# Fadi987/PL-BERT

Measured on AMD Instinct MI355X. Metric: phoneme-tokens/sec, higher is better.
Workload: dtype bf16; 1 GPU; PL-BERT masked-phoneme training step (fwd+loss+bwd+allreduce+AdamW), ALBERT hidden 768 / 12 shared layers / FFN 2048 / 12 heads, seq_len 512, batch 32 per GPU; global_batch=32, seq_len=512, parallelism=dp1

## Files before the change

### plbert_amd/_lib.py

```python
from __future__ import annotations

import ctypes as C
import os

import torch

HERE = os.path.dirname(os.path.abspath(__file__))
LIB_PATH = os.environ.get("PLBERT_HIP_LIB") or os.path.join(HERE, "libplbert_hip.so")

PLB_PARAM_NAMES = [
    "encoder.embeddings.word_embeddings.weight",
    "encoder.embeddings.position_embeddings.weight",
    "encoder.embeddings.token_type_embeddings.weight",
    "encoder.embeddings.LayerNorm.weight",
    "encoder.embeddings.LayerNorm.bias",
    "encoder.encoder.embedding_hidden_mapping_in.weight",
    "encoder.encoder.embedding_hidden_mapping_in.bias",
    "encoder.encoder.albert_layer_groups.0.albert_layers.0.full_layer_layer_norm.weight",
    "encoder.encoder.albert_layer_groups.0.albert_layers.0.full_layer_layer_norm.bias",
    "encoder.encoder.albert_layer_groups.0.albert_layers.0.attention.query.weight",
    "encoder.encoder.albert_layer_groups.0.albert_layers.0.attention.key.weight",
    "encoder.encoder.albert_layer_groups.0.albert_layers.0.attention.value.weight",
    "encoder.encoder.albert_layer_groups.0.albert_layers.0.attention.query.bias",
    "encoder.encoder.albert_layer_groups.0.albert_layers.0.attention.key.bias",
    "encoder.encoder.albert_layer_groups.0.albert_layers.0.attention.value.bias",
    "encoder.encoder.albert_layer_groups.0.albert_layers.0.attention.dense.weight",
    "encoder.encoder.albert_layer_groups.0.albert_layers.0.attention.dense.bias",
    "encoder.encoder.albert_layer_groups.0.albert_layers.0.attention.LayerNorm.weight",
    "encoder.encoder.albert_layer_groups.0.albert_layers.0.attention.LayerNorm.bias",
    "encoder.encoder.albert_layer_groups.0.albert_layers.0.ffn.weight",
    "encoder.encoder.albert_layer_groups.0.albert_layers.0.ffn.bias",
    "encoder.encoder.albert_layer_groups.0.albert_layers.0.ffn_output.weight",
    "encoder.encoder.albert_layer_groups.0.albert_layers.0.ffn_output.bias",
    "phoneme_predictor.weight",
    "phoneme_predictor.bias",
    "encoder.pooler.weight",
    "encoder.pooler.bias",
    "token_predictor.weight",
    "token_predictor.bias",
]
PLB_NPARAM = len(PLB_PARAM_NAMES)

PUBLIC_SYMBOLS = [
    "plb_last_error", "plb_create", "plb_destroy", "plb_param_layout", "plb_workspace_bytes", "plb_bind",
    "plb_sync_weights", "plb_forward", "plb_pooler", "plb_loss_fwd_bwd", "plb_loss_fwd", "plb_loss_fwd_bwd_dual", "plb_adamw_step",
    "plb_set_fp8", "plb_fp8_state", "plb_fp8_stats", "plb_token_head_steps", "plb_set_token_head_steps", "plb_comm_unique_id", "plb_comm_init", "plb_comm_destroy",
    "plb_comm_info", "plb_comm_pieces", "plb_last_application_rows", "plb_status", "plb_status_ex", "plb_poll_status", "plb_status_export", "plb_status_import", "plb_broadcast_params", "plb_set_grad_overlap", "plb_allreduce_grads", "plb_apply_mask",
    "plb_mask_batch", "plb_profile_enable", "plb_profile_num_classes", "plb_profile_class_name", "plb_profile_read",
    "plb_debug_skip_piece", "plb_debug_ln_fault", "plb_debug_hb_audit", "plb_debug_hb_report", "plb_comm_trace", "plb_comm_trace_read",
    "plb_set_gemm_nt_tile", "plb_set_gemm_nt_prefetch", "plb_set_attn_bwd_fused", "plb_set_prune_last",
]


class PlbConfig(C.Structure):
    _fields_ = [
        ("vocab_size", C.c_int32), ("embedding_size", C.c_int32), ("hidden_size", C.c_int32),
        ("num_attention_heads", C.c_int32), ("intermediate_size", C.c_int32), ("num_hidden_layers", C.c_int32),
        ("max_position_embeddings", C.c_int32), ("type_vocab_size", C.c_int32), ("layer_norm_eps", C.c_float),
        ("num_phonemes", C.c_int32), ("num_tokens", C.c_int32), ("max_batch", C.c_int32), ("max_seq", C.c_int32),
        ("inference_only", C.c_int32),
    ]


class PlbGemmNT(C.Structure):
    _fields_ = [
        ("A", C.c_void_p), ("lda", C.c_int), ("B", C.c_void_p), ("ldb", C.c_int),
        ("M", C.c_int), ("N", C.c_int), ("K", C.c_int), ("Mstore", C.c_int),
        ("bias", C.c_void_p), ("res", C.c_void_p), ("ldr", C.c_int), ("aux", C.c_void_p), ("ldaux", C.c_int),
        ("C", C.c_void_p), ("ldc", C.c_int), ("C2", C.c_void_p), ("ldc2", C.c_int), ("Cf", C.c_void_p), ("ldcf", C.c_int),
        ("colpart", C.c_void_p),
        ("ce_cols", C.c_int), ("ce_tgt", C.c_void_p), ("ce_pmax", C.c_void_p), ("ce_psum", C.c_void_p),
        ("ce_tlogit", C.c_void_p), ("ce_lse", C.c_void_p), ("ce_w", C.c_void_p),
        ("deq_a", C.c_void_p), ("deq_b", C.c_void_p), ("C8", C.c_void_p), ("ldc8", C.c_int), ("q_scale", C.c_void_p),
        ("q_amax", C.c_void_p), ("c8_bf8", C.c_int),
        ("ln_gamma", C.c_void_p), ("ln_beta", C.c_void_p), ("ln_mean", C.c_void_p), ("ln_rstd", C.c_void_p),
        ("ln_eps", C.c_float), ("ln_xchg", C.c_void_p), ("ln_err", C.c_void_p), ("ln_fault", C.c_int),
    ]


class PlbGemmTN(C.Structure):
    _fields_ = [
        ("A", C.c_void_p), ("lda", C.c_int), ("Ncols", C.c_int), ("B", C.c_void_p), ("ldb", C.c_int),
        ("Mtot", C.c_int), ("N", C.c_int), ("K", C.c_int), ("rows_per_split", C.c_int), ("splits", C.c_int),
        ("slab", C.c_void_p), ("deq_a", C.c_void_p), ("deq_b", C.c_void_p),
    ]


class PlbAttn(C.Structure):
    _fields_ = [
        ("qkv", C.c_void_p), ("ldqkv", C.c_int), ("lengths", C.c_void_p),
        ("B", C.c_int), ("S", C.c_int), ("NH", C.c_int), ("H", C.c_int), ("scale", C.c_float),
        ("ctx", C.c_void_p), ("ldctx", C.c_int), ("lse", C.c_void_p),
        ("dctx", C.c_void_p), ("lddctx", C.c_int), ("delta", C.c_void_p), ("dqkv", C.c_void_p), ("lddqkv", C.c_int),
        ("colpart", C.c_void_p), ("colpart_accumulate", C.c_int),
        ("ctx8", C.c_void_p), ("ldctx8", C.c_int), ("ctx_scale", C.c_void_p), ("ctx_amax", C.c_void_p),
        ("dqkv8", C.c_void_p), ("lddqkv8", C.c_int), ("dqkv_scale", C.c_void_p), ("dqkv_amax", C.c_void_p),
        ("qoff", C.c_void_p), ("q", C.c_void_p), ("ldq", C.c_int), ("nq_total", C.c_int), ("dq", C.c_void_p), ("lddq", C.c_int),
        ("dq8", C.c_void_p), ("lddq8", C.c_int),
    ]


class PlbEmbed(C.Structure):
    _fields_ = [
        ("ids", C.c_void_p), ("T", C.c_int), ("S", C.c_int), ("E", C.c_int), ("V", C.c_int),
        ("word", C.c_void_p), ("pos", C.c_void_p), ("type0", C.c_void_p), ("gamma", C.c_void_p), ("beta", C.c_void_p),
        ("eps", C.c_float), ("out", C.c_void_p), ("ldo", C.c_int), ("dout", C.c_void_p), ("lddo", C.c_int),
        ("dx", C.c_void_p), ("dword", C.c_void_p), ("dpos", C.c_void_p), ("partials", C.c_void_p), ("nblocks", C.c_int),
    ]


class PlbLayerNorm(C.Structure):
    _fields_ = [
        ("x", C.c_void_p), ("ldx", C.c_int), ("gamma", C.c_void_p), ("beta", C.c_void_p), ("eps", C.c_float),
        ("y", C.c_void_p), ("ldy", C.c_int), ("mean", C.c_void_p), ("rstd", C.c_void_p),
        ("T", C.c_int), ("H", C.c_int), ("Tzero", C.c_int),
        ("dy", C.c_void_p), ("lddy", C.c_int), ("dx", C.c_void_p), ("lddx", C.c_int),
        ("partials", C.c_void_p), ("nblocks", C.c_int), ("accumulate", C.c_int),
        ("out8", C.c_void_p), ("ld8", C.c_int), ("q_scale", C.c_void_p), ("q_amax", C.c_void_p),
    ]


_lib = None


class HipLibraryMissing(RuntimeError):
    pass


def lib():
    global _lib
    if _lib is not None:
        return _lib
    if not os.path.exists(LIB_PATH):
        raise HipLibraryMissing(
            f"{LIB_PATH} is missing: build it with `python -m plbert_amd.build` (needs hipcc, gfx950). "
            "There is no CPU fallback for the PL-BERT hot path.")
    try:
        L = C.CDLL(LIB_PATH, mode=C.RTLD_GLOBAL)
    except OSError as ex:
        raise HipLibraryMissing(f"cannot load {LIB_PATH}: {ex}") from ex
    vp, i32, i64p, f32, f64 = C.c_void_p, C.c_int32, C.POINTER(C.c_int64), C.c_float, C.c_double
    L.plb_last_error.restype = C.c_char_p
    L.plb_last_error.argtypes = []
    L.plb_create.restype = C.c_int
    L.plb_create.argtypes = [C.POINTER(PlbConfig), C.POINTER(vp)]
    L.plb_destroy.restype = None
    L.plb_destroy.argtypes = [vp]
    L.plb_param_layout.restype = C.c_int
    L.plb_param_layout.argtypes = [vp, i64p, i64p, i64p, i64p]
    L.plb_workspace_bytes.restype = C.c_int64
    L.plb_workspace_bytes.argtypes = [vp]
    L.plb_bind.restype = C.c_int
    L.plb_bind.argtypes = [vp, vp, vp, vp, vp, vp, C.c_int64]
    L.plb_sync_weights.restype = C.c_int
    L.plb_sync_weights.argtypes = [vp, vp]
    L.plb_forward.restype = C.c_int
    L.plb_forward.argtypes = [vp, vp, vp, i32, i32, vp, vp, vp, vp]
    L.plb_loss_fwd_bwd.restype = C.c_int
    L.plb_loss_fwd_bwd.argtypes = [vp, vp, vp, vp, vp, vp, i32, i32, i32, vp, vp]
    L.plb_loss_fwd_bwd_dual.restype = C.c_int
    L.plb_loss_fwd_bwd_dual.argtypes = [vp, vp, vp, vp, vp, vp, vp, i32, i32, i32, vp, vp, vp]
    L.plb_pooler.restype = C.c_int
    L.plb_pooler.argtypes = [vp, vp, i32, i32, vp, vp]
    L.plb_loss_fwd.restype = C.c_int
    L.plb_loss_fwd.argtypes = [vp, vp, vp, vp, vp, vp, vp, i32, i32, i32, vp, vp, vp]
    L.plb_set_fp8.restype = C.c_int
    L.plb_set_fp8.argtypes = [vp, i32, vp]
    L.plb_fp8_state.restype = C.c_int
    L.plb_fp8_state.argtypes = [vp, C.POINTER(i32), C.POINTER(i32)]
    L.plb_token_head_steps.restype = i32
    L.plb_token_head_steps.argtypes = [vp]
    L.plb_set_token_head_steps.restype = C.c_int
    L.plb_set_token_head_steps.argtypes = [vp, i32]
    L.plb_comm_unique_id.restype = C.c_int
    L.plb_comm_unique_id.argtypes = [vp]
    L.plb_comm_init.restype = C.c_int
    L.plb_comm_init.argtypes = [vp, vp, i32, i32]
    L.plb_comm_destroy.restype = C.c_int
    L.plb_comm_destroy.argtypes = [vp]
    L.plb_comm_info.restype = C.c_int
    L.plb_comm_info.argtypes = [vp, C.POINTER(i32), C.POINTER(i32), C.POINTER(i32)]
    L.plb_status.restype = C.c_int
    L.plb_status.argtypes = [vp, C.POINTER(i32)]
    L.plb_status_ex.restype = C.c_int
    L.plb_status_ex.argtypes = [vp, C.POINTER(i32), C.POINTER(i32)]
    L.plb_poll_status.restype = C.c_int
    L.plb_poll_status.argtypes = [vp, C.POINTER(i32)]
    L.plb_fp8_stats.restype = C.c_int
    L.plb_fp8_stats.argtypes = [vp, C.POINTER(f32), C.POINTER(f32), vp]
    L.plb_last_application_rows.restype = C.c_int
    L.plb_last_application_rows.argtypes = [vp, i64p, i64p]
    L.plb_status_export.restype = C.c_int
    L.plb_status_export.argtypes = [vp, vp, vp]
    L.plb_status_import.restype = C.c_int
    L.plb_status_import.argtypes = [vp, vp, vp]
    L.plb_debug_hb_audit.restype = C.c_int
    L.plb_debug_hb_audit.argtypes = [vp, i32, i32]
    L.plb_debug_hb_report.restype = C.c_int
    L.plb_debug_hb_report.argtypes = [vp, i64p, C.POINTER(i32), C.c_char_p, i32]
    L.plb_comm_trace.restype = C.c_int
    L.plb_comm_trace.argtypes = [vp, i32]
    L.plb_comm_trace_read.restype = C.c_int
    L.plb_comm_trace_read.argtypes = [vp, i32, C.POINTER(i32), i64p, i64p, C.POINTER(f32), C.POINTER(f32), C.POINTER(f32)]
    L.plb_debug_ln_fault.restype = None
    L.plb_debug_ln_fault.argtypes = [C.c_int, C.c_int]
    L.plb_debug_skip_piece.restype = None
    L.plb_debug_skip_piece.argtypes = [C.c_int]
    L.plb_comm_pieces.restype = C.c_int
    L.plb_comm_pieces.argtypes = [vp, C.POINTER(i32), C.POINTER(C.c_int64)]
    L.plb_broadcast_params.restype = C.c_int
    L.plb_broadcast_params.argtypes = [vp, i32, vp]
    L.plb_set_grad_overlap.restype = C.c_int
    L.plb_set_grad_overlap.argtypes = [vp, i32]
    L.plb_allreduce_grads.restype = C.c_int
    L.plb_allreduce_grads.argtypes = [vp, vp]
    L.plb_apply_mask.restype = C.c_int
    L.plb_apply_mask.argtypes = [vp, vp, vp, vp, vp, vp, vp, vp, C.c_int64, vp, i32, i32, i32, vp, vp, vp, vp, vp, vp, vp, vp]
    L.plb_adamw_step.restype = C.c_int
    L.plb_adamw_step.argtypes = [vp, f64, f64, f64, f64, f64, i32, f64, vp]
    L.plb_mask_batch.restype = C.c_int
    L.plb_mask_batch.argtypes = [vp, vp, i32, i32, C.c_uint64, C.c_uint32, f32, f32, f32, i32, i32, vp, vp, vp, vp, vp]
    L.plb_profile_enable.restype = None
    L.plb_profile_enable.argtypes = [C.c_int]
    L.plb_profile_num_classes.restype = C.c_int
    L.plb_profile_num_classes.argtypes = []
    L.plb_profile_class_name.restype = C.c_char_p
    L.plb_profile_class_name.argtypes = [C.c_int]
    L.plb_profile_read.restype = C.c_int
    L.plb_profile_read.argtypes = [C.POINTER(C.c_double), i64p, C.POINTER(C.c_double), C.POINTER(C.c_double)]
    L.plb_launch_gemm_nt.restype = C.c_int
    L.plb_launch_gemm_nt.argtypes = [C.POINTER(PlbGemmNT), C.c_int, C.c_int, vp]
    L.plb_set_gemm_nt_tile.restype = None
    L.plb_set_gemm_nt_tile.argtypes = [C.c_int]
    L.plb_set_gemm_nt_prefetch.restype = None
    L.plb_set_gemm_nt_prefetch.argtypes = [C.c_int]
    L.plb_launch_gemm_nt_fp8.restype = C.c_int
    L.plb_launch_gemm_nt_fp8.argtypes = [C.POINTER(PlbGemmNT), C.c_int, C.c_int, vp]
    L.plb_launch_gemm_nt_fp8_ln.restype = C.c_int
    L.plb_launch_gemm_nt_fp8_ln.argtypes = [C.POINTER(PlbGemmNT), C.c_int, C.c_int, vp]
    L.plb_launch_gemm_nt_fp8_gelud.restype = C.c_int
    L.plb_launch_gemm_nt_fp8_gelud.argtypes = [C.POINTER(PlbGemmNT), C.c_int, C.c_int, vp]
    L.plb_launch_gemm_tn.restype = C.c_int
    L.plb_launch_gemm_tn.argtypes = [C.POINTER(PlbGemmTN), vp]
    L.plb_launch_gemm_tn_big.restype = C.c_int
    L.plb_launch_gemm_tn_big.argtypes = [C.POINTER(PlbGemmTN), vp]
    L.plb_launch_gemm_tn_fp8.restype = C.c_int
    L.plb_launch_gemm_tn_fp8.argtypes = [C.POINTER(PlbGemmTN), vp]
    L.plb_launch_reduce_slabs.restype = C.c_int
    L.plb_launch_reduce_slabs.argtypes = [vp, C.c_int, C.c_size_t, vp, C.c_int, vp]
    L.plb_launch_attn_fwd.restype = C.c_int
    L.plb_launch_attn_fwd.argtypes = [C.POINTER(PlbAttn), vp]
    L.plb_launch_gemm_nt_ln.restype = C.c_int
    L.plb_launch_gemm_nt_ln.argtypes = [C.POINTER(PlbGemmNT), C.c_int, vp]
    L.plb_launch_gemm_nt_gelud.restype = C.c_int
    L.plb_launch_gemm_nt_gelud.argtypes = [C.POINTER(PlbGemmNT), C.c_int, vp]
    L.plb_launch_attn_bwd.restype = C.c_int
    L.plb_launch_attn_bwd.argtypes = [C.POINTER(PlbAttn), vp]
    L.plb_launch_attn_bwd_fused.restype = C.c_int
    L.plb_launch_attn_bwd_fused.argtypes = [C.POINTER(PlbAttn), vp]
    L.plb_set_prune_last.restype = None
    L.plb_set_prune_last.argtypes = [C.c_int]
    L.plb_set_attn_bwd_fused.restype = None
    L.plb_set_attn_bwd_fused.argtypes = [C.c_int]
    L.plb_launch_ln_fwd.restype = C.c_int
    L.plb_launch_ln_fwd.argtypes = [C.POINTER(PlbLayerNorm), vp]
    L.plb_launch_ln_bwd.restype = C.c_int
    L.plb_launch_ln_bwd.argtypes = [C.POINTER(PlbLayerNorm), vp]
    L.plb_launch_embed_scatter.restype = C.c_int
    L.plb_launch_embed_scatter.argtypes = [C.POINTER(PlbEmbed), C.c_int, vp]
    L.plb_launch_colsum.restype = C.c_int
    L.plb_launch_colsum.argtypes = [vp, C.c_int, C.c_size_t, C.c_int, C.c_int, vp, C.c_int, C.c_int, vp, C.c_int, vp]
    _lib = L
    return L


def profile_enable(on):
    lib().plb_profile_enable(int(bool(on)))


def profile_read():
    L = lib()
    n = L.plb_profile_num_classes()
    ms, fl, by = (C.c_double * n)(), (C.c_double * n)(), (C.c_double * n)()
    cnt = (C.c_int64 * n)()
    check(L.plb_profile_read(ms, cnt, fl, by), "plb_profile_read")
    return {L.plb_profile_class_name(i).decode(): dict(ms=ms[i], launches=int(cnt[i]), flops=fl[i], bytes=by[i])
            for i in range(n) if cnt[i]}


def check(rc, what):
    if rc != 0:
        msg = lib().plb_last_error().decode("utf-8", "replace")
        raise RuntimeError(f"{what} failed: {msg or 'rc=%d' % rc}")
```

### plbert_amd/build.py

```python
from __future__ import annotations

import os
import subprocess
import sys

HERE = os.path.dirname(os.path.abspath(__file__))
CSRC = os.path.join(HERE, "csrc")
LIB = os.path.join(HERE, "libplbert_hip.so")
SOURCES = ["gemm.hip", "gemm_big.hip", "gemm_fp8.hip", "gemm_fp8_ln.hip", "gemm_tn_fp8.hip", "gemm_ln.hip", "attn.hip", "attn_bwd_fused.hip", "rowops.hip", "mask.hip", "engine.cpp"]
HEADERS = ["common.h", "plbert_kernels.h", "gemm_epilogue.h", "gemm_nt_pipeline.h", "attn_common.h", os.path.join("..", "..", "include", "plbert.h")]
FLAGS = ["--offload-arch=gfx950", "-O3", "-std=c++17", "-fPIC", "-Wall", "-Wno-unused-function"]
_NO_SINK = ["-mllvm", "-disable-machine-sink"]
EXTRA_FLAGS = {"attn_bwd_fused.hip": ["-mllvm", "-amdgpu-mfma-vgpr-form=1"],
               "gemm_fp8.hip": _NO_SINK, "gemm_fp8_ln.hip": _NO_SINK, "gemm_tn_fp8.hip": _NO_SINK}


def _hipcc():
    for cand in (os.environ.get("HIPCC"), "/opt/rocm/bin/hipcc", "hipcc"):
        if cand and (os.path.isabs(cand) and os.path.exists(cand) or not os.path.isabs(cand)):
            return cand
    raise RuntimeError("hipcc not found")


def needs_build():
    if not os.path.exists(LIB):
        return True
    t = os.path.getmtime(LIB)
    deps = [os.path.join(CSRC, s) for s in SOURCES + HEADERS]
    return any(os.path.getmtime(d) > t for d in deps)


OBJDUMP = "/opt/rocm/lib/llvm/bin/llvm-objdump"


def disassemble_code_objects(lib, workdir):
    import glob
    import shutil
    cp = shutil.copy(lib, workdir)
    subprocess.run([OBJDUMP, "--offloading", cp], check=True, stdout=subprocess.PIPE, stderr=subprocess.STDOUT)
    cos = sorted(glob.glob(cp + ".*gfx950"))
    if not cos:
        raise RuntimeError("no gfx950 code object extracted from " + lib)
    for co in cos:
        yield co, subprocess.run([OBJDUMP, "-d", "--no-show-raw-insn", co], check=True, stdout=subprocess.PIPE,
                                 text=True).stdout


def verify_m0(lib=LIB, workdir=None):
    import re
    import tempfile
    if not os.path.exists(OBJDUMP):
        return None
    own = workdir is None
    tmp = tempfile.mkdtemp(prefix="plbert_m0_") if own else workdir
    n_asm = 0
    try:
        for co, text in disassemble_code_objects(lib, tmp):
            funcs, cur = {}, None
            for ln in text.splitlines():
                i = ln.split("//")[0].strip()
                m = re.match(r"^[0-9a-f]+ <(.+)>:$", i)
                if m:
                    cur = funcs.setdefault(m.group(1), [])
                elif cur is not None and i and not i.endswith(":"):
                    cur.append(i)
            for name, ins in funcs.items():
                def dma(i):
                    return i.startswith("global_load_lds") or (i.startswith("buffer_load") and i.rstrip().endswith("lds"))
                sig = [k for k in range(len(ins) - 2) if re.match(r"s_mov_b32 m0, s\d+$", ins[k]) and ins[k + 1] == "s_nop 0"
                       and dma(ins[k + 2]) and " s[" in ins[k + 2]]
                for i in ins:
                    if re.match(r"(s_movrel|v_movrel|ds_gws|ds_ordered|s_sendmsg|v_interp)", i):
                        raise RuntimeError(f"M0 check: {name}: instruction that reads M0: {i}")
                    if re.search(r"\bm0\b", i):
                        if not (re.match(r"s_\w+ m0, ", i) and not re.search(r"\bm0\b", i.split(",", 1)[1])):
                            raise RuntimeError(f"M0 check: {name}: M0 used as a source: {i}")
                if not sig:
                    continue
                n_asm += len(sig)
                owned = set(sig) | {k + 2 for k in sig}
                for k, i in enumerate(ins):
                    if (dma(i) or re.search(r"\bm0\b", i)) and k not in owned:
                        raise RuntimeError(f"M0 check: {name}: M0 / LDS-DMA outside the asm DMA statements: {ins[max(0, k - 2):k + 3]}")
    finally:
        if own:
            import shutil
            shutil.rmtree(tmp, ignore_errors=True)
    return n_asm


def build(force=False, verbose=True):
    if not force and not needs_build():
        return LIB
    hipcc = _hipcc()
    objdir = os.path.join(HERE, "build")
    os.makedirs(objdir, exist_ok=True)
    procs = []
    for src in SOURCES:
        obj = os.path.join(objdir, os.path.splitext(src)[0] + ".o")
        cmd = [hipcc, *FLAGS, *EXTRA_FLAGS.get(src, []), "-x", "hip", "-c", os.path.join(CSRC, src), "-o", obj]
        procs.append((src, obj, subprocess.Popen(cmd, stdout=subprocess.PIPE, stderr=subprocess.STDOUT, text=True)))
    objs = []
    for src, obj, p in procs:
        out, _ = p.communicate()
        if p.returncode != 0:
            raise RuntimeError(f"hipcc failed on {src}:\n{out}")
        if verbose and out.strip():
            print(out, file=sys.stderr)
        objs.append(obj)
    cmd = [hipcc, "--offload-arch=gfx950", "-shared", "-fPIC", "-o", LIB, *objs]
    r = subprocess.run(cmd, stdout=subprocess.PIPE, stderr=subprocess.STDOUT, text=True)
    if r.returncode != 0:
        raise RuntimeError("link failed:\n" + r.stdout)
    try:
        verify_m0(LIB)
    except Exception:
        os.remove(LIB)
        raise
    return LIB


if __name__ == "__main__":
    print(build(force="--force" in sys.argv))
```

### plbert_amd/csrc/gemm_ln.hip

```cpp
#include "gemm_nt_pipeline.h"

static int g_ln_fault_mode = 0, g_ln_fault_launches = 0;
extern "C" void plb_debug_ln_fault(int mode, int launches) { g_ln_fault_mode = mode; g_ln_fault_launches = launches; }
extern "C" int plb_ln_fault_take(void) {
  if (g_ln_fault_launches <= 0) return 0;
  --g_ln_fault_launches;
  return g_ln_fault_mode;
}

extern "C" int plb_launch_gemm_nt_ln(const PlbGemmNT* p_in, int mode, hipStream_t stream) {
  PlbGemmNT q_ = *p_in;
  q_.ln_fault = plb_ln_fault_take();
  const PlbGemmNT* p = &q_;
  if (mode != 5 && mode != 6) return 1;
  if (p->M % 1024 || p->K % 64 || p->M <= 0 || p->N <= 0 || p->K <= 0) return 3;
  const int tile = p->N % 384 == 0 ? 384 : p->N % 256 == 0 ? 256 : 0;
  if (!tile || p->N / tile > 4) return 3;
  if (!p->ln_gamma || !p->ln_mean || !p->ln_rstd || !p->ln_xchg || !p->ln_err || !p->C) return 1;
  if (mode == 5 && (!p->ln_beta || !p->C2)) return 1;
  if (mode == 6 && (!p->aux || !p->colpart)) return 1;
  if (p->res && (((uintptr_t)p->res & 15) || p->ldr % 8)) return 1;
  if (mode == 6 && (((uintptr_t)p->aux & 15) || p->ldaux % 8)) return 1;
  dim3 grid((p->M / 128) * (p->N / tile)), block(512);
  const double mnk = (double)p->M * p->N * p->K;
  const double bytes = 2.0 * ((double)p->M * p->K + (double)p->N * p->K) + (double)p->M * p->N * (mode == 5 ? 4 : 4) +
                       (p->res ? 2.0 * p->M * p->N : 0.0);
  const int tok = plb_prof_begin(mode == 5 ? PLB_K_GEMM_NT_LNFWD : PLB_K_GEMM_NT_LNBWD, stream, 2.0 * mnk, bytes);
  if (tile == 384) {
    if (mode == 5) hipLaunchKernelGGL((gemm_nt_big_kernel<3, 5, false, true>), grid, block, 0, stream, *p);
    else hipLaunchKernelGGL((gemm_nt_big_kernel<3, 6, false, true>), grid, block, 0, stream, *p);
  } else {
    if (mode == 5) hipLaunchKernelGGL((gemm_nt_big_kernel<1, 5, false, true>), grid, block, 0, stream, *p);
    else hipLaunchKernelGGL((gemm_nt_big_kernel<1, 6, false, true>), grid, block, 0, stream, *p);
  }
  plb_prof_end(tok, stream);
  return hipGetLastError() == hipSuccess ? 0 : 2;
}

extern "C" int plb_launch_gemm_nt_gelud(const PlbGemmNT* p, int backward, hipStream_t stream) {
  if (p->M % 256 || p->N % 256 || p->K % 64 || p->M <= 0 || p->N <= 0 || p->K <= 0) return 3;
  if (!p->C || (!backward && !p->C2) || (backward && !p->aux)) return 1;
  dim3 grid((p->M / 256) * (p->N / 256)), block(512);
  const double mnk = (double)p->M * p->N * p->K;
  const double bytes = 2.0 * ((double)p->M * p->K + (double)p->N * p->K) + 4.0 * p->M * p->N;
  const int tok = plb_prof_begin(backward ? PLB_K_GEMM_NT_GELUBWD : PLB_K_GEMM_NT_GELU, stream, 2.0 * mnk, bytes);
  if (backward) hipLaunchKernelGGL((gemm_nt_big_kernel<2, 8, false, true>), grid, block, 0, stream, *p);
  else if (p->colpart) hipLaunchKernelGGL((gemm_nt_big_kernel<2, 7, false, true>), grid, block, 0, stream, *p);
  else hipLaunchKernelGGL((gemm_nt_big_kernel<2, 7, false, true, false, false, true>), grid, block, 0, stream, *p);
  plb_prof_end(tok, stream);
  return hipGetLastError() == hipSuccess ? 0 : 2;
}
```

### plbert_amd/csrc/plbert_kernels.h

```cpp
#pragma once
#include <hip/hip_runtime.h>
#include <stdint.h>

typedef uint16_t bf16_t;

extern "C" {

enum PlbKernelClass {
  PLB_K_GEMM_NT = 0, PLB_K_GEMM_NT_GELU, PLB_K_GEMM_NT_GELUBWD, PLB_K_GEMM_NT_F32, PLB_K_GEMM_TN,
  PLB_K_ATTN_FWD, PLB_K_ATTN_BWD_DQ, PLB_K_ATTN_BWD_DKV, PLB_K_LN_FWD, PLB_K_LN_BWD, PLB_K_EMBED_FWD,
  PLB_K_EMBED_BWD, PLB_K_COLSUM, PLB_K_REDUCE, PLB_K_ROWS, PLB_K_CE, PLB_K_ADAMW, PLB_K_CAST, PLB_K_TOKEN_CE, PLB_K_GEMM_NT_CE, PLB_K_GEMM_NT_SMALL, PLB_K_FP8, PLB_K_ATTN_BWD,
  PLB_K_GEMM_NT_FP8, PLB_K_GEMM_NT_GELU_FP8, PLB_K_GEMM_NT_GELUBWD_FP8,
  PLB_K_GEMM_NT_LNFWD, PLB_K_GEMM_NT_LNBWD,
  PLB_K_GEMM_NT_LNFWD_FP8, PLB_K_GEMM_NT_LNBWD_FP8, PLB_K_GEMM_TN_FP8,
  PLB_K_NCLASS
};
int plb_prof_begin(int cls, hipStream_t s, double flops, double bytes);
void plb_prof_end(int tok, hipStream_t s);

typedef struct {
  const bf16_t* A; int lda;
  const bf16_t* B; int ldb;
  int M, N, K;
  int Mstore;
  const float* bias;
  const bf16_t* res; int ldr;
  const bf16_t* aux; int ldaux;
  bf16_t* C; int ldc;
  bf16_t* C2; int ldc2;
  float* Cf; int ldcf;
  float* colpart;
  int ce_cols;
  const int64_t* ce_tgt;
  float* ce_pmax; float* ce_psum;
  float* ce_tlogit;
  const float* ce_lse;
  const float* ce_w;
  const float* deq_a; const float* deq_b;
  uint8_t* C8; int ldc8;
  const float* q_scale;
  float* q_amax;
  int c8_bf8;
  const float* ln_gamma; const float* ln_beta;
  float* ln_mean; float* ln_rstd;
  float ln_eps;
  unsigned long long* ln_xchg;
  unsigned int* ln_err;
  int ln_fault;
} PlbGemmNT;
int plb_launch_gemm_nt_ln(const PlbGemmNT* p, int mode, hipStream_t stream);
int plb_launch_gemm_nt_gelud(const PlbGemmNT* p, int backward, hipStream_t stream);
int plb_launch_gemm_nt_fp8(const PlbGemmNT* p, int act, int a_bf8, hipStream_t stream);
int plb_launch_gemm_nt_fp8_ln(const PlbGemmNT* p, int mode, int a_bf8, hipStream_t stream);
int plb_launch_gemm_nt_fp8_gelud(const PlbGemmNT* p, int backward, int a_bf8, hipStream_t stream);
int plb_gemm_nt_fp8_gelud_tile_rows(int M);
int plb_ln_fault_take(void);
int plb_launch_gemm_nt(const PlbGemmNT* p, int act, int out_f32, hipStream_t stream);
int plb_gemm_nt_colpart_rows(int M, int N, int K);
void plb_set_gemm_nt_tile(int tile);
void plb_set_gemm_nt_prefetch(int on);

typedef struct {
  const bf16_t* A; int lda; int Ncols;
  const bf16_t* B; int ldb;
  int Mtot, N, K;
  int rows_per_split, splits;
  float* slab;
  const float* deq_a; const float* deq_b;
} PlbGemmTN;
int plb_launch_gemm_tn(const PlbGemmTN* p, hipStream_t stream);
int plb_launch_gemm_tn_fp8(const PlbGemmTN* p, hipStream_t stream);
int plb_launch_gemm_tn_big(const PlbGemmTN* p, hipStream_t stream);

int plb_launch_reduce_slabs(const float* slab, int splits, size_t n, float* out, int accumulate, hipStream_t stream);

typedef struct {
  const int64_t* ids; int T, S, E, V;
  const float *word, *pos, *type0, *gamma, *beta;
  float eps;
  bf16_t* out; int ldo;
  const bf16_t* dout; int lddo;
  float* dx;
  float *dword, *dpos;
  float* partials;
  int nblocks;
} PlbEmbed;
int plb_launch_embed_fwd(const PlbEmbed* p, hipStream_t stream);
int plb_launch_embed_bwd(const PlbEmbed* p, hipStream_t stream);
int plb_launch_embed_scatter(const PlbEmbed* p, int P, hipStream_t stream);

typedef struct {
  const bf16_t* x; int ldx;
  const float *gamma, *beta; float eps;
  bf16_t* y; int ldy;
  float *mean, *rstd;
  int T, H;
  int Tzero;
  const bf16_t* dy; int lddy;
  bf16_t* dx; int lddx;
  float* partials; int nblocks;
  int accumulate;
  uint8_t* out8; int ld8; const float* q_scale; float* q_amax;
} PlbLayerNorm;
int plb_launch_amax(const void* x, int is_bf16, size_t rows, int cols, int ld, float* amax, hipStream_t stream);
int plb_launch_fp8_scales(float* amax, float* scale, float* deq, int n, float fmax, int group, hipStream_t stream);
int plb_launch_fp8_scales2(float* amax, float* scale, float* deq, int n, float fmax, int group, int n2, float fmax2,
                           float* stats, int hist_from, hipStream_t stream);
int plb_launch_quantize(const void* x, int is_bf16, size_t rows, int cols, int ld, const float* scale, uint8_t* out, int ldo,
                        int bf8, hipStream_t stream);
int plb_launch_quantize_multi(int n, const void* const* src, const int* is_bf16, const size_t* elements,
                              const float* const* scale, uint8_t* const* dst, float* const* amax, hipStream_t stream);
int plb_launch_ln_fwd(const PlbLayerNorm* p, hipStream_t stream);
int plb_launch_ln_bwd(const PlbLayerNorm* p, hipStream_t stream);

int plb_launch_colsum(const void* X, int is_bf16, size_t R, int N, int ld, float* out, int Nout, int accumulate,
                      float* scratch, int nsplit, hipStream_t stream);

int plb_launch_copy_cols(const float* scratch, int nsplit, int N, int col0, int Nout, float* out, hipStream_t stream);

int plb_launch_pooler(const float* hidden, int B, int S, int H, const float* W, const float* bias, float* pooled,
                      hipStream_t stream);

typedef struct {
  const bf16_t* qkv; int ldqkv;
  const int32_t* lengths;
  int B, S, NH, H;
  float scale;
  bf16_t* ctx; int ldctx;
  float* lse;
  const bf16_t* dctx; int lddctx;
  float* delta;
  bf16_t* dqkv; int lddqkv;
  float* colpart;
  int colpart_accumulate;
  uint8_t* ctx8; int ldctx8; const float* ctx_scale; float* ctx_amax;
  uint8_t* dqkv8; int lddqkv8; const float* dqkv_scale; float* dqkv_amax;
  const int32_t* qoff; const bf16_t* q; int ldq; int nq_total; bf16_t* dq; int lddq; uint8_t* dq8; int lddq8;
} PlbAttn;
int plb_launch_attn_fwd(const PlbAttn* p, hipStream_t stream);
int plb_launch_attn_bwd(const PlbAttn* p, hipStream_t stream);
int plb_launch_attn_bwd_fused(const PlbAttn* p, hipStream_t stream);
void plb_debug_skip_piece(int index);
void plb_debug_ln_fault(int mode, int launches);
void plb_set_attn_bwd_fused(int on);

int plb_launch_gather_rows(const bf16_t* src, int lds_, const int32_t* rows, int n, int npad, int H, bf16_t* dst,
                           int ldd, hipStream_t stream);
int plb_launch_scatter_rows(const bf16_t* src, int lds_, const int32_t* rows, int n, int H, bf16_t* dst, int ldd,
                            hipStream_t stream);
int plb_launch_ce_prepare(const int32_t* offsets, const int32_t* flat, const int64_t* labels, int B, int S,
                          int32_t* rows, int32_t* tgt, float* w, hipStream_t stream);
int plb_launch_ce_fwd_bwd(const float* logits, int ldl, int V, const int32_t* tgt, const float* w, int n, int npad,
                          float* loss_rows, bf16_t* dlogits, int ldd, hipStream_t stream);
int plb_launch_sum_rows(const float* x, int n, float* out, hipStream_t stream);
int plb_launch_token_ce_combine(const float* pmax, const float* psum, int ntiles, const float* tlogit,
                                const int32_t* lengths, int B, int S, int rows, float* lse, float* w, float* loss_rows,
                                hipStream_t stream);
int plb_launch_add_scalar(float* out, const float* a, const float* b, hipStream_t stream);

typedef struct {
  const int64_t* labels; const int32_t* lengths;
  int B, S;
  uint64_t seed; uint32_t step;
  float word_pred_prob, mask_prob, replace_prob;
  int mask_id, sep_id;
  int64_t* masked; int32_t *counts, *idx_padded, *offsets, *flat;
} PlbMask;
int plb_launch_mask(const PlbMask* p, hipStream_t stream);

typedef struct {
  const int64_t* ids; const int32_t *sample_off, *word_off, *word_begin, *word_len; const int8_t* action;
  const int64_t* repl; const int64_t* word_token; int64_t sep_token; const int32_t* crop_start;
  int B, S, mask_id;
  int64_t *labels, *masked, *tokens; int32_t *lengths_out, *counts, *idx_padded, *offsets, *flat;
} PlbApplyMask;
int plb_launch_apply_mask(const PlbApplyMask* p, hipStream_t stream);

int plb_launch_adamw(float* p, const float* g, float* m, float* v, bf16_t* p_bf16, size_t n, double lr, double beta1,
                     double beta2, double eps, double wd, int step, double grad_scale, unsigned int* skip_if_nonzero,
                     int count_skip, hipStream_t stream);
int plb_launch_step_status(unsigned int* ln_err, float* loss, unsigned int* host_mirror, const float* summed, hipStream_t stream);
int plb_launch_status_export(const unsigned int* ln_err, float* out, hipStream_t stream);
int plb_launch_cast_bf16(const float* src, bf16_t* dst, size_t n, hipStream_t stream);
int plb_launch_transpose_cast(const float* src, int R, int C, bf16_t* dst, int ldd, hipStream_t stream);
int plb_launch_transpose_cast_multi(int n, const float* const* src, const int* R, const int* C, bf16_t* const* dst,
                                    const int* ldd, hipStream_t stream);
int plb_launch_bf16_to_f32(const bf16_t* src, int lds_, float* dst, int ldd, int R, int C, hipStream_t stream);

}
```

Baseline: 1.770 million tokens/s.

## Add ping-pong 128x256 NT GEMM kernel for GELU forward/backward

After: 1.775 million tokens/s, median of 6. Within noise of the previous version (+0.3%).

```diff
diff --git a/plbert_amd/_lib.py b/plbert_amd/_lib.py
--- a/plbert_amd/_lib.py
+++ b/plbert_amd/_lib.py
@@ -254,6 +254,8 @@
     L.plb_launch_gemm_nt_ln.argtypes = [C.POINTER(PlbGemmNT), C.c_int, vp]
     L.plb_launch_gemm_nt_gelud.restype = C.c_int
     L.plb_launch_gemm_nt_gelud.argtypes = [C.POINTER(PlbGemmNT), C.c_int, vp]
+    L.plb_set_nt_pingpong.restype = None
+    L.plb_set_nt_pingpong.argtypes = [C.c_int]
     L.plb_launch_attn_bwd.restype = C.c_int
     L.plb_launch_attn_bwd.argtypes = [C.POINTER(PlbAttn), vp]
     L.plb_launch_attn_bwd_fused.restype = C.c_int
diff --git a/plbert_amd/build.py b/plbert_amd/build.py
--- a/plbert_amd/build.py
+++ b/plbert_amd/build.py
@@ -8,7 +8,7 @@
 CSRC = os.path.join(HERE, "csrc")
 LIB = os.path.join(HERE, "libplbert_hip.so")
 SOURCES = ["gemm.hip", "gemm_big.hip", "gemm_fp8.hip", "gemm_fp8_ln.hip", "gemm_tn_fp8.hip", "gemm_ln.hip", "attn.hip", "attn_bwd_fused.hip", "rowops.hip", "mask.hip", "engine.cpp"]
-HEADERS = ["common.h", "plbert_kernels.h", "gemm_epilogue.h", "gemm_nt_pipeline.h", "attn_common.h", os.path.join("..", "..", "include", "plbert.h")]
+HEADERS = ["common.h", "plbert_kernels.h", "gemm_epilogue.h", "gemm_nt_pipeline.h", "gemm_nt_pair.h", "attn_common.h", os.path.join("..", "..", "include", "plbert.h")]
 FLAGS = ["--offload-arch=gfx950", "-O3", "-std=c++17", "-fPIC", "-Wall", "-Wno-unused-function"]
 _NO_SINK = ["-mllvm", "-disable-machine-sink"]
 EXTRA_FLAGS = {"attn_bwd_fused.hip": ["-mllvm", "-amdgpu-mfma-vgpr-form=1"],
diff --git a/plbert_amd/csrc/gemm_ln.hip b/plbert_amd/csrc/gemm_ln.hip
--- a/plbert_amd/csrc/gemm_ln.hip
+++ b/plbert_amd/csrc/gemm_ln.hip
@@ -1,4 +1,8 @@
 #include "gemm_nt_pipeline.h"
+#include "gemm_nt_pair.h"
+
+#include <cstdlib>
+#include <cstring>
 
 static int g_ln_fault_mode = 0, g_ln_fault_launches = 0;
 extern "C" void plb_debug_ln_fault(int mode, int launches) { g_ln_fault_mode = mode; g_ln_fault_launches = launches; }
@@ -37,13 +41,27 @@
   return hipGetLastError() == hipSuccess ? 0 : 2;
 }
 
+static int g_nt_pingpong = -1;
+extern "C" void plb_set_nt_pingpong(int on) { g_nt_pingpong = on; }
+static bool nt_pingpong() {
+  static const bool env = [] { const char* e = getenv("PLBERT_NT_PINGPONG"); return !(e && !strcmp(e, "0")); }();
+  return g_nt_pingpong < 0 ? env : g_nt_pingpong != 0;
+}
 extern "C" int plb_launch_gemm_nt_gelud(const PlbGemmNT* p, int backward, hipStream_t stream) {
   if (p->M % 256 || p->N % 256 || p->K % 64 || p->M <= 0 || p->N <= 0 || p->K <= 0) return 3;
   if (!p->C || (!backward && !p->C2) || (backward && !p->aux)) return 1;
-  dim3 grid((p->M / 256) * (p->N / 256)), block(512);
   const double mnk = (double)p->M * p->N * p->K;
   const double bytes = 2.0 * ((double)p->M * p->K + (double)p->N * p->K) + 4.0 * p->M * p->N;
   const int tok = plb_prof_begin(backward ? PLB_K_GEMM_NT_GELUBWD : PLB_K_GEMM_NT_GELU, stream, 2.0 * mnk, bytes);
+  if (nt_pingpong() && !p->res) {
+    dim3 grid((p->M / 128) * (p->N / 256)), block(256);
+    if (backward) hipLaunchKernelGGL((gemm_nt_pair_kernel<8, false>), grid, block, 0, stream, *p);
+    else if (p->colpart) hipLaunchKernelGGL((gemm_nt_pair_kernel<7, false>), grid, block, 0, stream, *p);
+    else hipLaunchKernelGGL((gemm_nt_pair_kernel<7, true>), grid, block, 0, stream, *p);
+    plb_prof_end(tok, stream);
+    return hipGetLastError() == hipSuccess ? 0 : 2;
+  }
+  dim3 grid((p->M / 256) * (p->N / 256)), block(512);
   if (backward) hipLaunchKernelGGL((gemm_nt_big_kernel<2, 8, false, true>), grid, block, 0, stream, *p);
   else if (p->colpart) hipLaunchKernelGGL((gemm_nt_big_kernel<2, 7, false, true>), grid, block, 0, stream, *p);
   else hipLaunchKernelGGL((gemm_nt_big_kernel<2, 7, false, true, false, false, true>), grid, block, 0, stream, *p);
diff --git a/plbert_amd/csrc/gemm_nt_pair.h b/plbert_amd/csrc/gemm_nt_pair.h
--- /dev/null
+++ b/plbert_amd/csrc/gemm_nt_pair.h
@@ -0,0 +1,235 @@
+#pragma once
+#include "gemm_nt_pipeline.h"
+
+namespace {
+
+constexpr int PR_HT = 128 * 64;
+constexpr int PR_RING = 5;
+DEVI int pr_slot(int x) { return x >= PR_RING ? x - PR_RING : x; }
+
+#define PR_BARRIER()                             \
+  do {                                           \
+    __builtin_amdgcn_s_waitcnt(0xC07F);          \
+    asm volatile("s_barrier" ::: "memory");      \
+  } while (0)
+#define PR_PIN() __builtin_amdgcn_sched_barrier(0)
+
+template <int ACT, bool NOCS>
+__global__ __launch_bounds__(256, 2) void gemm_nt_pair_kernel(PlbGemmNT p) {
+  static_assert(ACT == 7 || ACT == 8, "gelu forms only");
+  constexpr int TM = 128, TN = 256;
+  __shared__ __attribute__((aligned(16))) bf16_t smem[PR_RING * PR_HT];
+  const int tid = threadIdx.x, lane = tid & 63;
+  const int wn = __builtin_amdgcn_readfirstlane(tid >> 6);
+  const int nbn = p.N / TN;
+  const int logical = xcd_remap(blockIdx.x, gridDim.x);
+  const int bm = logical / nbn, bn = logical % nbn;
+  const int b256 = bm >> 1, wm = bm & 1;
+  const int nk = p.K / 64;
+
+  const int drow = lane >> 3;
+  const int ch0 = ((lane & 7) ^ ((lane >> 4) & 7)) * 16;
+  const int ch1 = ((lane & 7) ^ ((4 + (lane >> 4)) & 7)) * 16;
+  uint32_t vA[4], vB[4];
+#pragma unroll
+  for (int j = 0; j < 4; ++j) {
+    vA[j] = (uint32_t)((((4 * wn + j) >> 3) * 128 + ((4 * wn + j) & 7) * 8 + drow) * p.lda * 2 + ((j & 1) ? ch1 : ch0));
+    vB[j] = (uint32_t)(((4 * wn + j) * 8 + drow) * p.ldb * 2 + ((j & 1) ? ch1 : ch0));
+  }
+  const char* const sA_ = (const char*)p.A + (size_t)(b256 * 256 + wm * 64) * p.lda * 2;
+  const char* const sB_ = (const char*)p.B + (size_t)(bn * TN) * p.ldb * 2;
+  const size_t hB = (size_t)128 * p.ldb * 2;
+  const uint32_t ldsb_ = LDS_ADDR(&smem[0]);
+#define PR_DMA(h, j)                                                                                          \
+  do {                                                                                                        \
+    const int t_ = (h) / 3, i_ = (h) - 3 * ((h) / 3);                                                         \
+    const uint32_t d_ = ldsb_ + 2u * (pr_slot((h) % PR_RING) * PR_HT + (4 * wn + (j)) * 8 * 64);              \
+    if (i_ == 0) DMA16(sA_ + (size_t)t_ * 128, vA[j], d_);                                                    \
+    else DMA16(sB_ + (i_ - 1) * hB + (size_t)t_ * 128, vB[j], d_);                                            \
+  } while (0)
+#define PR_IS(h, j) do { if ((h) < htot) PR_DMA(h, j); PR_PIN(); } while (0)
+
+  const int frow = lane & 15, fq = lane >> 4;
+  const int fsw = (frow >> 1) & 7;
+  const int offA = frow * 64, offB = (wn * 32 + frow) * 64;
+  const int c0 = ((0 + fq) ^ fsw) << 3, c1 = ((4 + fq) ^ fsw) << 3;
+  bf16x8 afr[8][2], bfr[2][2][2];
+  f32x4 acc[8][2][2];
+#pragma unroll
+  for (int s = 0; s < 8; ++s)
+#pragma unroll
+    for (int nh = 0; nh < 2; ++nh)
+#pragma unroll
+      for (int ni = 0; ni < 2; ++ni) acc[s][nh][ni] = f32x4{0.f, 0.f, 0.f, 0.f};
+#define PR_RA(slot, s, kk) \
+  do { afr[s][kk] = *(const bf16x8*)&smem[(slot) * PR_HT + offA + (s) * 16 * 64 + ((kk) ? c1 : c0)]; PR_PIN(); } while (0)
+#define PR_RB(nh, slot, ni, kk) \
+  do { bfr[nh][ni][kk] = *(const bf16x8*)&smem[(slot) * PR_HT + offB + (ni) * 16 * 64 + ((kk) ? c1 : c0)]; PR_PIN(); } while (0)
+#define PR_MF(nh, j)                                                                                          \
+  do {                                                                                                        \
+    acc[((j) >> 1) & 7][nh][(j) & 1] = __builtin_amdgcn_mfma_f32_16x16x32_bf16(                               \
+        bfr[nh][(j) & 1][(j) >> 4], afr[((j) >> 1) & 7][(j) >> 4], acc[((j) >> 1) & 7][nh][(j) & 1], 0, 0, 0); \
+    PR_PIN();                                                                                                 \
+  } while (0)
+#define PR_LANDED(need, issued)                                                                               \
+  do {                                                                                                        \
+    const int f_ = (issued) - (need);                                                                         \
+    if (f_ >= 2) asm volatile("s_waitcnt vmcnt(8)" ::: "memory");                                             \
+    else if (f_ == 1) asm volatile("s_waitcnt vmcnt(4)" ::: "memory");                                        \
+    else asm volatile("s_waitcnt vmcnt(0)" ::: "memory");                                                     \
+  } while (0)
+
+  const int htot = 3 * nk;
+#pragma unroll
+  for (int h = 0; h < PR_RING; ++h)
+#pragma unroll
+    for (int j = 0; j < 4; ++j) PR_IS(h, j);
+  PR_LANDED(3, htot < PR_RING ? htot : PR_RING);
+  PR_BARRIER();
+#pragma unroll
+  for (int s = 0; s < 8; ++s) { PR_RA(0, s, 0); PR_RA(0, s, 1); }
+#pragma unroll
+  for (int ni = 0; ni < 2; ++ni) { PR_RB(0, 1, ni, 0); PR_RB(0, 1, ni, 1); }
+  int rb = 0;
+  for (int t = 0; t < nk; ++t) {
+    const int h0 = 3 * t;
+    const int sB1 = pr_slot(rb + 2), sA = pr_slot(rb + 3), sB0 = pr_slot(rb + 4);
+    PR_BARRIER(); PR_PIN();
+    PR_MF(0, 0);  PR_RB(1, sB1, 0, 0); PR_MF(0, 1);  PR_IS(h0 + 5, 0); PR_MF(0, 2);  PR_RB(1, sB1, 0, 1); PR_MF(0, 3);
+    PR_IS(h0 + 5, 1); PR_MF(0, 4);  PR_RB(1, sB1, 1, 0); PR_MF(0, 5);  PR_IS(h0 + 5, 2); PR_MF(0, 6);
+    PR_RB(1, sB1, 1, 1); PR_MF(0, 7);  PR_IS(h0 + 5, 3); PR_MF(0, 8);  PR_MF(0, 9);  PR_IS(h0 + 6, 0); PR_MF(0, 10);
+    PR_MF(0, 11); PR_IS(h0 + 6, 1); PR_MF(0, 12); PR_MF(0, 13); PR_IS(h0 + 6, 2); PR_MF(0, 14); PR_MF(0, 15);
+    PR_IS(h0 + 6, 3); PR_MF(0, 16); PR_MF(0, 17); PR_MF(0, 18); PR_MF(0, 19); PR_MF(0, 20); PR_MF(0, 21); PR_MF(0, 22);
+    PR_MF(0, 23); PR_MF(0, 24); PR_MF(0, 25); PR_MF(0, 26); PR_MF(0, 27); PR_MF(0, 28); PR_MF(0, 29); PR_MF(0, 30);
+    PR_MF(0, 31);
+    PR_LANDED(h0 + 5, h0 + 7 < htot ? h0 + 7 : htot);
+    PR_BARRIER(); PR_PIN();
+    PR_MF(1, 0);  PR_RB(0, sB0, 0, 0); PR_MF(1, 1);  PR_RA(sA, 0, 0); PR_MF(1, 2);  PR_RB(0, sB0, 0, 1);
+    PR_MF(1, 3);  PR_RA(sA, 1, 0); PR_MF(1, 4);  PR_RB(0, sB0, 1, 0); PR_MF(1, 5);  PR_RA(sA, 2, 0);
+    PR_MF(1, 6);  PR_RB(0, sB0, 1, 1); PR_MF(1, 7);  PR_RA(sA, 3, 0); PR_MF(1, 8);  PR_IS(h0 + 7, 0);
+    PR_MF(1, 9);  PR_RA(sA, 4, 0); PR_MF(1, 10); PR_IS(h0 + 7, 1); PR_MF(1, 11); PR_RA(sA, 5, 0);
+    PR_MF(1, 12); PR_IS(h0 + 7, 2); PR_MF(1, 13); PR_RA(sA, 6, 0); PR_MF(1, 14); PR_IS(h0 + 7, 3);
+    PR_MF(1, 15); PR_RA(sA, 7, 0); PR_MF(1, 16); PR_MF(1, 17); PR_RA(sA, 0, 1); PR_MF(1, 18); PR_MF(1, 19);
+    PR_RA(sA, 1, 1); PR_MF(1, 20); PR_MF(1, 21); PR_RA(sA, 2, 1); PR_MF(1, 22); PR_MF(1, 23); PR_RA(sA, 3, 1);
+    PR_MF(1, 24); PR_MF(1, 25); PR_RA(sA, 4, 1); PR_MF(1, 26); PR_MF(1, 27); PR_RA(sA, 5, 1); PR_MF(1, 28);
+    PR_MF(1, 29); PR_RA(sA, 6, 1); PR_MF(1, 30); PR_MF(1, 31); PR_RA(sA, 7, 1);
+    if (t + 1 < nk) PR_LANDED(h0 + 6, h0 + 8 < htot ? h0 + 8 : htot);
+    rb = pr_slot(rb + 3);
+  }
+  PR_BARRIER();
+#undef PR_DMA
+#undef PR_IS
+#undef PR_RA
+#undef PR_RB
+#undef PR_MF
+#undef PR_LANDED
+
+  constexpr int OROW = TN + 8;
+  static_assert(TM * OROW <= PR_RING * PR_HT, "output image must fit the ring");
+  f32x4 csum[2][2];
+  float4 bz[2][2];
+#pragma unroll
+  for (int nh = 0; nh < 2; ++nh)
+#pragma unroll
+    for (int ni = 0; ni < 2; ++ni) {
+      csum[nh][ni] = f32x4{0.f, 0.f, 0.f, 0.f};
+      bz[nh][ni] = p.bias ? *(const float4*)(p.bias + bn * TN + nh * 128 + wn * 32 + ni * 16 + fq * 4)
+                          : make_float4(0.f, 0.f, 0.f, 0.f);
+    }
+  const int ncol0 = bn * TN + wn * 32 + fq * 4;
+  uint4* const lane_stash = reinterpret_cast<uint4*>(ACT == 7 ? p.C : const_cast<bf16_t*>(p.aux));
+  const size_t stash0 = (size_t)(b256 * nbn + bn) * 16 * 512 + lane + 64 * (wm * 4 + wn);
+#define PR_STASH(s, nh) (stash0 + (size_t)((s) * 2 + (nh)) * 512)
+  constexpr int SQD = 3;
+  uint4 sq[SQD + 1][2];
+#pragma unroll
+  for (int s = 0; s < 8; ++s) {
+    const int lrow = (s >> 2) * 64 + (s & 3) * 16 + frow;
+    const int m = b256 * 256 + (s >> 2) * 128 + wm * 64 + (s & 3) * 16 + frow;
+    uint2 ux[2][2];
+    if constexpr (ACT == 8) {
+      if (s == 0) {
+#pragma unroll
+        for (int a = 0; a < SQD; ++a)
+#pragma unroll
+          for (int nh = 0; nh < 2; ++nh) sq[a][nh] = lane_stash[PR_STASH(a, nh)];
+      }
+      if (s + SQD < 8) {
+#pragma unroll
+        for (int nh = 0; nh < 2; ++nh) sq[(s + SQD) % (SQD + 1)][nh] = lane_stash[PR_STASH(s + SQD, nh)];
+      }
+#pragma unroll
+      for (int nh = 0; nh < 2; ++nh) {
+        const uint4 q = sq[s % (SQD + 1)][nh];
+        ux[nh][0] = make_uint2(q.x, q.y); ux[nh][1] = make_uint2(q.z, q.w);
+      }
+    }
+    const bool st = m < p.Mstore;
+    uint2 dpair = make_uint2(0u, 0u);
+#pragma unroll
+    for (int nh = 0; nh < 2; ++nh)
+#pragma unroll
+      for (int ni = 0; ni < 2; ++ni) {
+        f32x4 v = acc[s][nh][ni];
+        v[0] += bz[nh][ni].x; v[1] += bz[nh][ni].y; v[2] += bz[nh][ni].z; v[3] += bz[nh][ni].w;
+        if constexpr (ACT == 8) {
+          v[0] = v[0] != 0.f ? v[0] * bf_lo(ux[nh][ni].x) : 0.f; v[1] = v[1] != 0.f ? v[1] * bf_hi(ux[nh][ni].x) : 0.f;
+          v[2] = v[2] != 0.f ? v[2] * bf_lo(ux[nh][ni].y) : 0.f; v[3] = v[3] != 0.f ? v[3] * bf_hi(ux[nh][ni].y) : 0.f;
+        }
+        uint2 gpk = make_uint2(0u, 0u);
+        if constexpr (ACT == 7) {
+          f32x4 gg;
+#pragma unroll
+          for (int r = 0; r < 4; ++r) {
+            const float x = v[r], x2 = x * x;
+            const float sg = gelu_sigmoid(x, x2);
+            gg[r] = x * sg;
+            v[r] = __builtin_fmaf(sg, x * __builtin_fmaf(x2, 0.21406444f, 1.5957691f) * (1.0f - sg), sg);
+          }
+          gpk.x = pack_bf2(gg[0], gg[1]); gpk.y = pack_bf2(gg[2], gg[3]);
+          asm volatile("" : "+v"(gpk.x), "+v"(gpk.y));
+        }
+        uint2 o; o.x = pack_bf2(v[0], v[1]); o.y = pack_bf2(v[2], v[3]);
+        if constexpr (ACT == 7) {
+          if (ni == 0) dpair = o;
+          else __builtin_nontemporal_store(u32x4nt{dpair.x, dpair.y, o.x, o.y}, (u32x4nt*)(lane_stash + PR_STASH(s, nh)));
+          *(uint2*)&smem[lrow * OROW + nh * 128 + wn * 32 + ni * 16 + fq * 4] = gpk;
+        } else {
+          *(uint2*)&smem[lrow * OROW + nh * 128 + wn * 32 + ni * 16 + fq * 4] = o;
+        }
+        v = f32x4{bf_lo(o.x), bf_hi(o.x), bf_lo(o.y), bf_hi(o.y)};
+        if (!NOCS && st) csum[nh][ni] += v;
+      }
+  }
+#undef PR_STASH
+  {
+    constexpr int CPR = TN / 8;
+    const int ldimg = ACT == 7 ? p.ldc2 : p.ldc;
+    bf16_t* const cbase = (ACT == 7 ? p.C2 : p.C) + (size_t)(b256 * 256 + wm * 64) * ldimg + bn * TN;
+    const int rows_ok = p.Mstore - (b256 * 256 + wm * 64);
+    __syncthreads();
+#pragma unroll 4
+    for (int c = tid; c < TM * CPR; c += 256) {
+      const int r = c / CPR, cc = c - r * CPR;
+      const int gr = (r >> 6) * 128 + (r & 63);
+      const uint4 v = *(const uint4*)&smem[r * OROW + cc * 8];
+      if (gr < rows_ok) __builtin_nontemporal_store(u32x4nt{v.x, v.y, v.z, v.w}, (u32x4nt*)(cbase + (size_t)gr * ldimg + cc * 8));
+    }
+  }
+  if (!NOCS && p.colpart) {
+#pragma unroll
+    for (int nh = 0; nh < 2; ++nh)
+#pragma unroll
+      for (int ni = 0; ni < 2; ++ni) {
+        f32x4 v = csum[nh][ni];
+        v = f32x4{row16_sum(v[0]), row16_sum(v[1]), row16_sum(v[2]), row16_sum(v[3])};
+        if (frow == 0)
+          *(float4*)(p.colpart + (size_t)bm * p.N + ncol0 + nh * 128 + ni * 16) = make_float4(v[0], v[1], v[2], v[3]);
+      }
+  }
+}
+
+#undef PR_BARRIER
+#undef PR_PIN
+
+}
diff --git a/plbert_amd/csrc/plbert_kernels.h b/plbert_amd/csrc/plbert_kernels.h
--- a/plbert_amd/csrc/plbert_kernels.h
+++ b/plbert_amd/csrc/plbert_kernels.h
@@ -50,6 +50,7 @@
 } PlbGemmNT;
 int plb_launch_gemm_nt_ln(const PlbGemmNT* p, int mode, hipStream_t stream);
 int plb_launch_gemm_nt_gelud(const PlbGemmNT* p, int backward, hipStream_t stream);
+void plb_set_nt_pingpong(int on);
 int plb_launch_gemm_nt_fp8(const PlbGemmNT* p, int act, int a_bf8, hipStream_t stream);
 int plb_launch_gemm_nt_fp8_ln(const PlbGemmNT* p, int mode, int a_bf8, hipStream_t stream);
 int plb_launch_gemm_nt_fp8_gelud(const PlbGemmNT* p, int backward, int a_bf8, hipStream_t stream);
```
